# JohannesErnst/WeaSAL

Hardware: AMD Instinct MI355X
Metric: points/sec fwd+bwd KPFCNN on DALES spheres; achieved HBM GB/s on KPConv gather (higher is better)
Workload: dtype f32; 1 GPU; DALES_PseudoLabel KP-FCNN, in_radius=10m, 50k pts/sphere, batch=8, fp32, step = GPU pyramid + fwd + loss + bwd + SGD; contrast_loss term included (trainer_PseudoLabel.py:204-208); pyramid of the next batch overlapped on a second stream; parallelism=dp1, dist_world_size=1, allreduce_bytes=0

## Files before the change

### weasal_amd/csrc/pools.hip

```cpp
#include "ws_common.h"
#include <algorithm>
#include "ws_dispatch.h"

namespace {

__device__ __forceinline__ int64_t ws_ceil_div_dev(int64_t a, int64_t b) { return (a + b - 1) / b; }
bool al16p(const void* p) { return (reinterpret_cast<uintptr_t>(p) & 15u) == 0; }
__device__ __forceinline__ int4 load_arg4(const int32_t* p) { return *reinterpret_cast<const int4*>(p); }
__device__ __forceinline__ int4 load_arg4(const uint8_t* p)
{
    const unsigned w = *reinterpret_cast<const unsigned*>(p);
    return make_int4((int)(w & 0xffu), (int)((w >> 8) & 0xffu), (int)((w >> 16) & 0xffu), (int)(w >> 24));
}

__device__ __forceinline__ void pool_groups(int64_t ngroups, int ilv, int wave, int64_t& g0, int64_t& gstep, int64_t& gend)
{
    if (ilv > 0 && (gridDim.x & 7) == 0) {
        const int x = blockIdx.x & 7, lb = blockIdx.x >> 3, nbx = gridDim.x >> 3;
        const int64_t per8 = (ngroups + 7) / 8;
        const int64_t b8 = (int64_t)x * per8;
        gend = b8 + per8 < ngroups ? b8 + per8 : ngroups;
        g0 = b8 + (int64_t)lb * 4 + wave;
        gstep = (int64_t)nbx * 4;
    } else {
        int64_t ibeg, iend;
        ws_block_range(ngroups, ibeg, iend);
        g0 = ibeg + wave; gstep = 4; gend = iend;
    }
}

template <int G, typename T, typename AT = int32_t, int U = 4>
__global__ __launch_bounds__(256) void max_pool_fwd_vec_kernel(const T* __restrict__ x, int64_t ns, int c,
                                                                const int64_t* __restrict__ inds, int64_t nq, int h,
                                                                T* __restrict__ out, AT* __restrict__ arg,
                                                                const int32_t* __restrict__ order = nullptr, int ilv = 0, int split = 1)
{
    constexpr int S = 64 / G;
    const int wave = __builtin_amdgcn_readfirstlane(threadIdx.x >> 6), lane = threadIdx.x & 63;
    const int j = lane % G, slot = lane / G;
    int64_t g0, gstep, gend;
    pool_groups(ws_ceil_div_dev(nq, S) * split, ilv, wave, g0, gstep, gend);
    for (int64_t grp = g0; grp < gend; grp += gstep) {
        const int64_t qi = (grp / split) * S + slot;
        const bool qok = qi < nq;
        const int64_t q = (qok && order) ? (int64_t)order[qi] : qi;
        const int cbeg = split > 1 ? (int)(grp % split) * (4 * G) : 0;
        const int cend = split > 1 ? min(cbeg + 4 * G, c) : c;
        for (int c0 = cbeg; c0 < cend; c0 += 4 * G) {
            const int ch = c0 + 4 * j;
            const bool ok = qok && ch < c;
            float4 best = make_float4(-3.4e38f, -3.4e38f, -3.4e38f, -3.4e38f);
            int bi[4] = {0, 0, 0, 0};
            for (int h0 = 0; h0 < h; h0 += U) {
                float4 v[U];
#pragma unroll
                for (int u = 0; u < U; ++u) {
                    v[u] = make_float4(0.f, 0.f, 0.f, 0.f);
                    const int col = h0 + u;
                    int64_t s = (ok && col < h) ? inds[q * h + col] : -1;
                    if (s >= 0 && s < ns) v[u] = ld4(x + s * c + ch);
                    else if (col >= h) v[u] = make_float4(-3.4e38f, -3.4e38f, -3.4e38f, -3.4e38f);
                }
#pragma unroll
                for (int u = 0; u < U; ++u) {
                    if (v[u].x > best.x) { best.x = v[u].x; bi[0] = h0 + u; }
                    if (v[u].y > best.y) { best.y = v[u].y; bi[1] = h0 + u; }
                    if (v[u].z > best.z) { best.z = v[u].z; bi[2] = h0 + u; }
                    if (v[u].w > best.w) { best.w = v[u].w; bi[3] = h0 + u; }
                }
            }
            if (ok) {
                st4(out + q * c + ch, best);
                if (arg) {
                    if constexpr (sizeof(AT) == 4)
                        *reinterpret_cast<int4*>(arg + q * c + ch) = make_int4(bi[0], bi[1], bi[2], bi[3]);
                    else
                        *reinterpret_cast<unsigned*>(arg + q * c + ch) =
                            (unsigned)bi[0] | ((unsigned)bi[1] << 8) | ((unsigned)bi[2] << 16) | ((unsigned)bi[3] << 24);
                }
            }
        }
    }
}

template <typename T>
__global__ __launch_bounds__(256) void max_pool_fwd_kernel(const T* __restrict__ x, int64_t ns, int c,
                                                            const int64_t* __restrict__ inds, int64_t nq, int h,
                                                            T* __restrict__ out, int32_t* __restrict__ arg)
{
    const int wave = __builtin_amdgcn_readfirstlane(threadIdx.x >> 6), lane = threadIdx.x & 63;
    for (int64_t q = (int64_t)blockIdx.x * 4 + wave; q < nq; q += (int64_t)gridDim.x * 4) {
        for (int c0 = 0; c0 < c; c0 += 64) {
            const int ch = c0 + lane;
            float best = -3.4e38f;
            int bi = 0;
            for (int j = 0; j < h; ++j) {
                const int64_t s = inds[q * h + j];
                float v = 0.0f;
                if (s >= 0 && s < ns && ch < c) v = ld1(x + s * c + ch);
                if (v > best) { best = v; bi = j; }
            }
            if (ch < c) {
                st1(out + q * c + ch, best);
                if (arg) arg[q * c + ch] = bi;
            }
        }
    }
}

template <int G, typename T, typename AT = int32_t>
__global__ __launch_bounds__(256) void max_pool_bwd_vec_kernel(const T* __restrict__ dy, const AT* __restrict__ arg,
                                                                int h, int c, const int32_t* __restrict__ t_offsets,
                                                                const int32_t* __restrict__ t_pairs, int64_t ns,
                                                                T* __restrict__ dx, const int32_t* __restrict__ order = nullptr,
                                                                int ilv = 0, const T* __restrict__ add = nullptr, int split = 1)
{
    constexpr int S = 64 / G;
    const int wave = __builtin_amdgcn_readfirstlane(threadIdx.x >> 6), lane = threadIdx.x & 63;
    const int j = lane % G, slot = lane / G;
    int64_t g0, gstep, gend;
    pool_groups(ws_ceil_div_dev(ns, S) * split, ilv, wave, g0, gstep, gend);
    for (int64_t grp = g0; grp < gend; grp += gstep) {
        const int64_t si = (grp / split) * S + slot;
        const bool sok = si < ns;
        const int64_t s = (sok && order) ? (int64_t)order[si] : si;
        const int beg = sok ? t_offsets[s] : 0, end = sok ? t_offsets[s + 1] : 0;
        const int cbeg = split > 1 ? (int)(grp % split) * (4 * G) : 0;
        const int cend = split > 1 ? min(cbeg + 4 * G, c) : c;
        for (int c0 = cbeg; c0 < cend; c0 += 4 * G) {
            const int ch = c0 + 4 * j;
            if (!(sok && ch < c)) continue;
            float4 acc = make_float4(0.f, 0.f, 0.f, 0.f);
            int p = beg;
            for (; p + 3 < end; p += 4) {
                int q4[4], col4[4];
                int4 a4[4];
#pragma unroll
                for (int u = 0; u < 4; ++u) {
                    const int pair = t_pairs[p + u];
                    q4[u] = pair / h;
                    col4[u] = pair - q4[u] * h;
                }
#pragma unroll
                for (int u = 0; u < 4; ++u) a4[u] = load_arg4(arg + (int64_t)q4[u] * c + ch);
#pragma unroll
                for (int u = 0; u < 4; ++u) {
                    const int4 a = a4[u];
                    const int col = col4[u];
                    if (a.x == col || a.y == col || a.z == col || a.w == col) {
                        const float4 g = ld4(dy + (int64_t)q4[u] * c + ch);
                        if (a.x == col) acc.x += g.x;
                        if (a.y == col) acc.y += g.y;
                        if (a.z == col) acc.z += g.z;
                        if (a.w == col) acc.w += g.w;
                    }
                }
            }
            for (; p < end; ++p) {
                const int pair = t_pairs[p];
                const int q = pair / h, col = pair - q * h;
                const int4 a = load_arg4(arg + (int64_t)q * c + ch);
                if (a.x == col || a.y == col || a.z == col || a.w == col) {
                    const float4 g = ld4(dy + (int64_t)q * c + ch);
                    if (a.x == col) acc.x += g.x;
                    if (a.y == col) acc.y += g.y;
                    if (a.z == col) acc.z += g.z;
                    if (a.w == col) acc.w += g.w;
                }
            }
            if (add) { const float4 o = ld4(add + s * c + ch); acc.x += o.x; acc.y += o.y; acc.z += o.z; acc.w += o.w; }
            st4(dx + s * c + ch, acc);
        }
    }
}

template <typename T>
__global__ __launch_bounds__(256) void max_pool_bwd_kernel(const T* __restrict__ dy, const int32_t* __restrict__ arg,
                                                            int h, int c, const int32_t* __restrict__ t_offsets,
                                                            const int32_t* __restrict__ t_pairs, int64_t ns,
                                                            T* __restrict__ dx)
{
    const int wave = __builtin_amdgcn_readfirstlane(threadIdx.x >> 6), lane = threadIdx.x & 63;
    for (int64_t s = (int64_t)blockIdx.x * 4 + wave; s < ns; s += (int64_t)gridDim.x * 4) {
        const int beg = t_offsets[s], end = t_offsets[s + 1];
        for (int c0 = 0; c0 < c; c0 += 64) {
            const int ch = c0 + lane;
            float acc = 0.0f;
            if (ch < c) {
                for (int p = beg; p < end; ++p) {
                    const int pair = t_pairs[p];
                    const int q = pair / h, col = pair - q * h;
                    if (arg[(int64_t)q * c + ch] == col) acc += ld1(dy + (int64_t)q * c + ch);
                }
                st1(dx + s * c + ch, acc);
            }
        }
    }
}

template <typename T>
__global__ __launch_bounds__(256) void closest_pool_fwd_kernel(const T* __restrict__ x, int64_t ns, int c,
                                                                const int64_t* __restrict__ inds, int64_t nq, int h,
                                                                T* __restrict__ out)
{
    const int wave = __builtin_amdgcn_readfirstlane(threadIdx.x >> 6), lane = threadIdx.x & 63;
    for (int64_t q = (int64_t)blockIdx.x * 4 + wave; q < nq; q += (int64_t)gridDim.x * 4) {
        const int64_t s = inds[q * h];
        const bool real = s >= 0 && s < ns;
        for (int ch = lane; ch < c; ch += 64) st1(out + q * c + ch, real ? ld1(x + s * c + ch) : 0.0f);
    }
}

template <typename T>
__global__ __launch_bounds__(256) void closest_pool_bwd_kernel(const T* __restrict__ dy, int h, int c,
                                                                const int32_t* __restrict__ t_offsets,
                                                                const int32_t* __restrict__ t_pairs, int64_t ns,
                                                                T* __restrict__ dx)
{
    const int wave = __builtin_amdgcn_readfirstlane(threadIdx.x >> 6), lane = threadIdx.x & 63;
    for (int64_t s = (int64_t)blockIdx.x * 4 + wave; s < ns; s += (int64_t)gridDim.x * 4) {
        const int beg = t_offsets[s], end = t_offsets[s + 1];
        for (int c0 = 0; c0 < c; c0 += 64) {
            const int ch = c0 + lane;
            float acc = 0.0f;
            if (ch < c) {
                for (int p = beg; p < end; ++p) {
                    const int pair = t_pairs[p];
                    const int q = pair / h;
                    if (pair - q * h == 0) acc += ld1(dy + (int64_t)q * c + ch);
                }
                st1(dx + s * c + ch, acc);
            }
        }
    }
}


template <int G>
__global__ __launch_bounds__(256) void closest_pool_bwd_vec_kernel(const float* __restrict__ dy, int h, int c,
                                                                    const int32_t* __restrict__ t_offsets,
                                                                    const int32_t* __restrict__ t_pairs, int64_t ns,
                                                                    float* __restrict__ dx)
{
    constexpr int S = 64 / G;
    const int wave = __builtin_amdgcn_readfirstlane(threadIdx.x >> 6), lane = threadIdx.x & 63;
    const int j = lane % G, slot = lane / G;
    for (int64_t s = (int64_t)blockIdx.x * 4 + wave; s < ns; s += (int64_t)gridDim.x * 4) {
        const int beg = t_offsets[s], end = t_offsets[s + 1];
        for (int c0 = 0; c0 < c; c0 += 4 * G) {
            const int ch = c0 + 4 * j;
            float4 acc = make_float4(0.f, 0.f, 0.f, 0.f);
            int p = beg + slot;
            for (; p + S < end; p += 2 * S) {
                const int pa = t_pairs[p], pb = t_pairs[p + S];
                const int qa = pa / h, qb = pb / h;
                float4 a = make_float4(0.f, 0.f, 0.f, 0.f), b4 = a;
                if (pa - qa * h == 0) a = *reinterpret_cast<const float4*>(dy + (int64_t)qa * c + ch);
                if (pb - qb * h == 0) b4 = *reinterpret_cast<const float4*>(dy + (int64_t)qb * c + ch);
                acc.x += a.x; acc.y += a.y; acc.z += a.z; acc.w += a.w;
                acc.x += b4.x; acc.y += b4.y; acc.z += b4.z; acc.w += b4.w;
            }
            if (p < end) {
                const int pa = t_pairs[p];
                const int qa = pa / h;
                if (pa - qa * h == 0) {
                    const float4 a = *reinterpret_cast<const float4*>(dy + (int64_t)qa * c + ch);
                    acc.x += a.x; acc.y += a.y; acc.z += a.z; acc.w += a.w;
                }
            }
#pragma unroll
            for (int o = G; o < 64; o <<= 1) {
                acc.x += __shfl_xor(acc.x, o, 64); acc.y += __shfl_xor(acc.y, o, 64);
                acc.z += __shfl_xor(acc.z, o, 64); acc.w += __shfl_xor(acc.w, o, 64);
            }
            if (slot == 0) *reinterpret_cast<float4*>(dx + s * c + ch) = acc;
        }
    }
}

constexpr int POOL_INTERLEAVE = 256;
constexpr int POOL_SPLIT_ROWS = 8192;
extern "C" int ws_closest_bwd_vec = 1;

enum { PK_MAX_FWD_VEC, PK_MAX_FWD, PK_MAX_BWD_VEC, PK_MAX_BWD, PK_CLOSEST_FWD, PK_CLOSEST_BWD, PK_CLOSEST_BWD_VEC };
struct PoolPlan {
    int kernel;
    bool bf16;
    int g;
    int u;
    int arg_bytes;
    int split;
    int ilv;
    int grid;
};
const char* row_name(const PoolPlan& p) { return p.bf16 ? "bf16" : "f32"; }

int pool_grid(int64_t groups, int ilv)
{
    if (ilv <= 0) return ws_grid(groups, 4);
    const int64_t need = (groups + 31) / 32;
    return 8 * (int)std::max<int64_t>(1, std::min<int64_t>(ilv, need));
}

PoolPlan max_pool_plan(bool fwd, bool bf16, int64_t rows, int c, const void* a, const void* b, const void* arg, int arg_bytes, bool ordered)
{
    PoolPlan p{fwd ? PK_MAX_FWD : PK_MAX_BWD, bf16, 0, 0, arg_bytes, 1, 0, ws_grid(rows, 4)};
    const bool rows_al = bf16 ? ws_row_aligned<bf16_t>(a) && ws_row_aligned<bf16_t>(b) : ws_row_aligned<float>(a) && ws_row_aligned<float>(b);
    if (arg_bytes != 1 && !(c % 4 == 0 && rows_al && al16p(arg))) return p;
    p.kernel = fwd ? PK_MAX_FWD_VEC : PK_MAX_BWD_VEC;
    p.g = (fwd && c <= 16) ? 4 : (c <= 32 ? 8 : (c <= 64 ? 16 : (c <= 128 ? 32 : 64)));
    p.u = (fwd && arg_bytes == 1 && p.g == 32) ? 8 : 4;
    p.split = (rows < POOL_SPLIT_ROWS && c > 256) ? (int)ws_ceil_div(c, 256) : 1;
    p.ilv = ordered ? POOL_INTERLEAVE : 0;
    p.grid = pool_grid(ws_ceil_div(rows, 64 / p.g) * p.split, p.ilv);
    return p;
}

PoolPlan closest_fwd_plan(bool bf16, int64_t nq) { return PoolPlan{PK_CLOSEST_FWD, bf16, 0, 0, 0, 1, 0, ws_grid(nq, 4)}; }

PoolPlan closest_bwd_plan(bool bf16, int64_t ns, int c, const void* dy, const void* dx)
{
    PoolPlan p{PK_CLOSEST_BWD, bf16, 0, 0, 0, 1, 0, ws_grid(ns, 4)};
    if (!bf16 && ws_closest_bwd_vec && al16p(dy) && al16p(dx) && (c == 32 || c == 64 || c == 128 || c % 256 == 0)) {
        p.kernel = PK_CLOSEST_BWD_VEC;
        p.g = c % 256 == 0 ? 64 : c / 4;
    }
    return p;
}

void plan_text(const PoolPlan& p, char* out, size_t n)
{
    const char* op = (p.kernel == PK_MAX_FWD_VEC || p.kernel == PK_MAX_FWD) ? "max_fwd" : "max_bwd";
    switch (p.kernel) {
    case PK_MAX_FWD_VEC: case PK_MAX_BWD_VEC:
        snprintf(out, n, "%s vec G=%d U=%d AT=%s %s split=%d %s", op, p.g, p.u, p.arg_bytes == 1 ? "u8" : "i32", row_name(p), p.split,
                 p.ilv ? "interleaved" : "contiguous");
        break;
    case PK_MAX_FWD: case PK_MAX_BWD: snprintf(out, n, "%s generic %s", op, row_name(p)); break;
    case PK_CLOSEST_FWD: snprintf(out, n, "closest_fwd scalar %s", row_name(p)); break;
    case PK_CLOSEST_BWD: snprintf(out, n, "closest_bwd scalar %s", row_name(p)); break;
    default: snprintf(out, n, "closest_bwd vec G=%d", p.g);
    }
}

int launched(bool hit, const PoolPlan& p)
{
    if (!hit) return ws_no_instantiation("pool kernel family %d <G=%d, U=%d> bf16=%d arg_bytes=%d", p.kernel, p.g, p.u, p.bf16, p.arg_bytes);
    WS_LAUNCH_CHECK();
    return WS_OK;
}

int launch_fwd(const PoolPlan& p, void* stream, const void* x, int64_t ns, int32_t c, const int64_t* inds, int64_t nq, int32_t h, void* out,
               void* arg, const int32_t* order)
{
    hipStream_t st = (hipStream_t)stream;
    bool hit = false;
    if (p.kernel == PK_MAX_FWD_VEC)
        dispatch([&](auto bf, auto g, auto u, auto u8) {
            using T = Row<bf.value>;
            using AT = std::conditional_t<u8.value != 0, uint8_t, int32_t>;
            if constexpr (!(bf.value && u8.value) && (u.value == 8) == (u8.value && g.value == 32)) {
                max_pool_fwd_vec_kernel<g.value, T, AT, u.value><<<p.grid, 256, 0, st>>>((const T*)x, ns, c, inds, nq, h, (T*)out, (AT*)arg, order,
                                                                                         p.ilv, p.split);
                hit = true;
            }
        }, Flag{p.bf16}, Pick<4, 8, 16, 32, 64>{p.g}, Pick<4, 8>{p.u}, Flag{p.arg_bytes == 1});
    else
        hit = dispatch([&](auto bf) {
            using T = Row<bf.value>;
            if (p.kernel == PK_MAX_FWD) max_pool_fwd_kernel<T><<<p.grid, 256, 0, st>>>((const T*)x, ns, c, inds, nq, h, (T*)out, (int32_t*)arg);
            else closest_pool_fwd_kernel<T><<<p.grid, 256, 0, st>>>((const T*)x, ns, c, inds, nq, h, (T*)out);
        }, Flag{p.bf16});
    return launched(hit, p);
}

int launch_bwd(const PoolPlan& p, void* stream, const void* dy, const void* arg, int32_t h, int32_t c, const int32_t* t_offsets,
               const int32_t* t_pairs, int64_t ns, void* dx, const int32_t* order, const float* add = nullptr)
{
    hipStream_t st = (hipStream_t)stream;
    bool hit = false;
    if (p.kernel == PK_MAX_BWD_VEC)
        dispatch([&](auto bf, auto g, auto u8) {
            using T = Row<bf.value>;
            using AT = std::conditional_t<u8.value != 0, uint8_t, int32_t>;
            if constexpr (!(bf.value && u8.value)) {
                max_pool_bwd_vec_kernel<g.value, T, AT><<<p.grid, 256, 0, st>>>((const T*)dy, (const AT*)arg, h, c, t_offsets, t_pairs, ns, (T*)dx,
                                                                                order, p.ilv, (const T*)add, p.split);
                hit = true;
            }
        }, Flag{p.bf16}, Pick<8, 16, 32, 64>{p.g}, Flag{p.arg_bytes == 1});
    else if (p.kernel == PK_CLOSEST_BWD_VEC)
        hit = dispatch([&](auto g) {
            closest_pool_bwd_vec_kernel<g.value><<<p.grid, 256, 0, st>>>((const float*)dy, h, c, t_offsets, t_pairs, ns, (float*)dx);
        }, Pick<8, 16, 32, 64>{p.g});
    else
        hit = dispatch([&](auto bf) {
            using T = Row<bf.value>;
            if (p.kernel == PK_MAX_BWD) max_pool_bwd_kernel<T><<<p.grid, 256, 0, st>>>((const T*)dy, (const int32_t*)arg, h, c, t_offsets, t_pairs, ns, (T*)dx);
            else closest_pool_bwd_kernel<T><<<p.grid, 256, 0, st>>>((const T*)dy, h, c, t_offsets, t_pairs, ns, (T*)dx);
        }, Flag{p.bf16});
    return launched(hit, p);
}

int pool_fwd_impl(bool closest, bool bf16, const void* x, int64_t ns, int32_t c, const int64_t* inds, int64_t nq, int32_t h, void* out,
                  int32_t* arg, const int32_t* order, void* stream)
{
    WS_REQUIRE(ns >= 0 && nq >= 0 && c >= 1 && h >= 1, "bad sizes");
    if (nq == 0) return WS_OK;
    WS_REQUIRE(inds && out && (ns == 0 || x), "NULL argument");
    const PoolPlan p = closest ? closest_fwd_plan(bf16, nq) : max_pool_plan(true, bf16, nq, c, x, out, arg, 4, order != nullptr);
    return launch_fwd(p, stream, x, ns, c, inds, nq, h, out, arg, order);
}

int pool_bwd_impl(bool closest, bool bf16, const void* dy, const int32_t* arg, int64_t nq, int32_t h, int32_t c, const int32_t* t_offsets,
                  const int32_t* t_pairs, int64_t ns, void* dx, const int32_t* order, void* stream)
{
    WS_REQUIRE(ns >= 0 && nq >= 0 && c >= 1 && h >= 1, "bad sizes");
    if (ns == 0) return WS_OK;
    WS_REQUIRE(t_offsets && dx && (nq == 0 || (dy && (closest || arg) && t_pairs)), "NULL argument");
    const PoolPlan p = closest ? closest_bwd_plan(bf16, ns, c, dy, dx) : max_pool_plan(false, bf16, ns, c, dy, dx, arg, 4, order != nullptr);
    return launch_bwd(p, stream, dy, arg, h, c, t_offsets, t_pairs, ns, dx, order);
}

}

extern "C" {

int ws_max_pool_fwd(const float* x, int64_t ns, int32_t c, const int64_t* inds, int64_t nq, int32_t h,
                    float* out, int32_t* arg, void* stream)
{
    return pool_fwd_impl(false, false, x, ns, c, inds, nq, h, out, arg, nullptr, stream);
}

int ws_max_pool_bwd(const float* dy, const int32_t* arg, int64_t nq, int32_t h, int32_t c,
                    const int32_t* t_offsets, const int32_t* t_pairs, int64_t ns, float* dx, void* stream)
{
    return pool_bwd_impl(false, false, dy, arg, nq, h, c, t_offsets, t_pairs, ns, dx, nullptr, stream);
}

int ws_max_pool_fwd_ordered(const float* x, int64_t ns, int32_t c, const int64_t* inds, int64_t nq, int32_t h, float* out, int32_t* arg,
                            const int32_t* order_q, void* stream)
{
    return pool_fwd_impl(false, false, x, ns, c, inds, nq, h, out, arg, order_q, stream);
}

int ws_max_pool_bwd_ordered(const float* dy, const int32_t* arg, int64_t nq, int32_t h, int32_t c, const int32_t* t_offsets,
                            const int32_t* t_pairs, int64_t ns, float* dx, const int32_t* order_s, void* stream)
{
    return pool_bwd_impl(false, false, dy, arg, nq, h, c, t_offsets, t_pairs, ns, dx, order_s, stream);
}

int ws_max_pool_fwd_ordered_bf16(const uint16_t* x, int64_t ns, int32_t c, const int64_t* inds, int64_t nq, int32_t h, uint16_t* out,
                                 int32_t* arg, const int32_t* order_q, void* stream)
{
    return pool_fwd_impl(false, true, x, ns, c, inds, nq, h, out, arg, order_q, stream);
}

int ws_max_pool_bwd_ordered_bf16(const uint16_t* dy, const int32_t* arg, int64_t nq, int32_t h, int32_t c, const int32_t* t_offsets,
                                 const int32_t* t_pairs, int64_t ns, uint16_t* dx, const int32_t* order_s, void* stream)
{
    return pool_bwd_impl(false, true, dy, arg, nq, h, c, t_offsets, t_pairs, ns, dx, order_s, stream);
}

int ws_closest_pool_fwd(const float* x, int64_t ns, int32_t c, const int64_t* inds, int64_t nq, int32_t h,
                        float* out, void* stream)
{
    return pool_fwd_impl(true, false, x, ns, c, inds, nq, h, out, nullptr, nullptr, stream);
}

int ws_closest_pool_bwd(const float* dy, int64_t nq, int32_t h, int32_t c, const int32_t* t_offsets,
                        const int32_t* t_pairs, int64_t ns, float* dx, void* stream)
{
    return pool_bwd_impl(true, false, dy, nullptr, nq, h, c, t_offsets, t_pairs, ns, dx, nullptr, stream);
}

int ws_max_pool_fwd_bf16(const uint16_t* x, int64_t ns, int32_t c, const int64_t* inds, int64_t nq, int32_t h,
                         uint16_t* out, int32_t* arg, void* stream)
{
    return pool_fwd_impl(false, true, x, ns, c, inds, nq, h, out, arg, nullptr, stream);
}

int ws_max_pool_bwd_bf16(const uint16_t* dy, const int32_t* arg, int64_t nq, int32_t h, int32_t c,
                         const int32_t* t_offsets, const int32_t* t_pairs, int64_t ns, uint16_t* dx, void* stream)
{
    return pool_bwd_impl(false, true, dy, arg, nq, h, c, t_offsets, t_pairs, ns, dx, nullptr, stream);
}

int ws_closest_pool_fwd_bf16(const uint16_t* x, int64_t ns, int32_t c, const int64_t* inds, int64_t nq, int32_t h,
                             uint16_t* out, void* stream)
{
    return pool_fwd_impl(true, true, x, ns, c, inds, nq, h, out, nullptr, nullptr, stream);
}

int ws_closest_pool_bwd_bf16(const uint16_t* dy, int64_t nq, int32_t h, int32_t c, const int32_t* t_offsets,
                             const int32_t* t_pairs, int64_t ns, uint16_t* dx, void* stream)
{
    return pool_bwd_impl(true, true, dy, nullptr, nq, h, c, t_offsets, t_pairs, ns, dx, nullptr, stream);
}

int ws_priv_max_pool_fwd_u8(const float* x, int64_t ns, int32_t c, const int64_t* inds, int64_t nq, int32_t h, float* out,
                            uint8_t* arg, const int32_t* order_q, void* stream)
{
    if (nq == 0) return WS_OK;
    return launch_fwd(max_pool_plan(true, false, nq, c, x, out, arg, 1, order_q != nullptr), stream, x, ns, c, inds, nq, h, out, arg, order_q);
}

int ws_priv_max_pool_bwd_u8(const float* dy, const uint8_t* arg, int64_t nq, int32_t h, int32_t c, const int32_t* t_offsets,
                            const int32_t* t_pairs, int64_t ns, float* dx, const int32_t* order_s, const float* add, void* stream)
{
    (void)nq;
    if (ns == 0) return WS_OK;
    return launch_bwd(max_pool_plan(false, false, ns, c, dy, dx, arg, 1, order_s != nullptr), stream, dy, arg, h, c, t_offsets, t_pairs, ns,
                          dx, order_s, add);
}

int ws_pool_variant(int32_t op, int64_t rows, int32_t c, const void* rows_a, const void* rows_b, const void* arg, int32_t rows_bf16,
                    int32_t arg_bytes, int32_t ordered, char* out, int32_t cap, int32_t* grid)
{
    WS_REQUIRE(out && cap > 0 && rows >= 0 && c >= 1 && (arg_bytes == 4 || arg_bytes == 1), "bad argument");
    const bool bf = rows_bf16 != 0, max_op = op == WS_POOL_MAX_FWD || op == WS_POOL_MAX_BWD;
    WS_REQUIRE(arg_bytes == 4 || (max_op && !bf && c % 4 == 0 && al16p(rows_a) && al16p(rows_b) && (reinterpret_cast<uintptr_t>(arg) & 3u) == 0),
               "the byte arg-max record: max-pools of f32 rows, c %% 4 == 0, 16-byte aligned rows, 4-byte aligned arg");
    PoolPlan p;
    switch (op) {
    case WS_POOL_MAX_FWD: case WS_POOL_MAX_BWD: p = max_pool_plan(op == WS_POOL_MAX_FWD, bf, rows, c, rows_a, rows_b, arg, arg_bytes, ordered != 0); break;
    case WS_POOL_CLOSEST_FWD: p = closest_fwd_plan(bf, rows); break;
    case WS_POOL_CLOSEST_BWD: p = closest_bwd_plan(bf, rows, c, rows_a, rows_b); break;
    default: return ws_fail(WS_ERR_INVALID, "unknown pool operation %d", op);
    }
    plan_text(p, out, (size_t)cap);
    if (grid) *grid = p.grid;
    return WS_OK;
}

}
```

Before: 32.61 million points/s.

## Software-pipeline pair/offset loads and shuffle-broadcast pairs in pool backward kernels

Result: no change. 32.88 million points/s (median of 3 runs) (+0.8%).

```diff
diff --git a/weasal_amd/csrc/pools.hip b/weasal_amd/csrc/pools.hip
--- a/weasal_amd/csrc/pools.hip
+++ b/weasal_amd/csrc/pools.hip
@@ -6,12 +6,6 @@
 
 __device__ __forceinline__ int64_t ws_ceil_div_dev(int64_t a, int64_t b) { return (a + b - 1) / b; }
 bool al16p(const void* p) { return (reinterpret_cast<uintptr_t>(p) & 15u) == 0; }
-__device__ __forceinline__ int4 load_arg4(const int32_t* p) { return *reinterpret_cast<const int4*>(p); }
-__device__ __forceinline__ int4 load_arg4(const uint8_t* p)
-{
-    const unsigned w = *reinterpret_cast<const unsigned*>(p);
-    return make_int4((int)(w & 0xffu), (int)((w >> 8) & 0xffu), (int)((w >> 16) & 0xffu), (int)(w >> 24));
-}
 
 __device__ __forceinline__ void pool_groups(int64_t ngroups, int ilv, int wave, int64_t& g0, int64_t& gstep, int64_t& gend)
 {
@@ -108,69 +102,112 @@
     }
 }
 
-template <int G, typename T, typename AT = int32_t>
+__device__ __forceinline__ int4 load_argp(const int32_t* p) { return *reinterpret_cast<const int4*>(p); }
+__device__ __forceinline__ unsigned load_argp(const uint8_t* p) { return *reinterpret_cast<const unsigned*>(p); }
+__device__ __forceinline__ int argp_ch(const int4& a, int i) { return i == 0 ? a.x : (i == 1 ? a.y : (i == 2 ? a.z : a.w)); }
+__device__ __forceinline__ int argp_ch(unsigned w, int i) { return (int)((w >> (8 * i)) & 0xffu); }
+template <typename P>
+__device__ __forceinline__ bool argp_any(const P& a, int col)
+{
+    return argp_ch(a, 0) == col || argp_ch(a, 1) == col || argp_ch(a, 2) == col || argp_ch(a, 3) == col;
+}
+__device__ __forceinline__ void split_pair(int pair, int h, int& q, int& col)
+{
+    q = 0; col = -1;
+    if (pair >= 0) { q = pair / h; col = pair - q * h; }
+}
+
+constexpr int POOL_BWD_BATCH = 4;
+
+template <int G, typename T, typename AT = int32_t, int B = (sizeof(AT) == 1 ? POOL_BWD_BATCH : POOL_BWD_BATCH / 2)>
 __global__ __launch_bounds__(256) void max_pool_bwd_vec_kernel(const T* __restrict__ dy, const AT* __restrict__ arg,
                                                                 int h, int c, const int32_t* __restrict__ t_offsets,
                                                                 const int32_t* __restrict__ t_pairs, int64_t ns,
                                                                 T* __restrict__ dx, const int32_t* __restrict__ order = nullptr,
                                                                 int ilv = 0, const T* __restrict__ add = nullptr, int split = 1)
 {
+    static_assert(G % B == 0, "a batch never straddles a pair chunk");
     constexpr int S = 64 / G;
     const int wave = __builtin_amdgcn_readfirstlane(threadIdx.x >> 6), lane = threadIdx.x & 63;
     const int j = lane % G, slot = lane / G;
     int64_t g0, gstep, gend;
     pool_groups(ws_ceil_div_dev(ns, S) * split, ilv, wave, g0, gstep, gend);
+
+    auto slot_si = [&](int64_t g) -> int64_t {
+        const int64_t si = (split > 1 ? g / split : g) * S + slot;
+        return (g < gend && si < ns) ? si : -1;
+    };
+    auto ld_order = [&](int64_t g) -> int { const int64_t si = slot_si(g); return (order && si >= 0) ? order[si] : 0; };
+    auto row_of = [&](int64_t g, int ov) -> int64_t { const int64_t si = slot_si(g); return (order && si >= 0) ? (int64_t)ov : si; };
+    auto ld_offsets = [&](int64_t s, int& b, int& e) { b = e = 0; if (s >= 0) { b = t_offsets[s]; e = t_offsets[s + 1]; } };
+    auto ld_chunk = [&](int b, int e, int k0) -> int { return k0 + j < e - b ? t_pairs[b + k0 + j] : -1; };
+
+    int o0 = ld_order(g0), o1 = ld_order(g0 + gstep), o2 = ld_order(g0 + 2 * gstep);
+    int b0, e0, b1, e1;
+    ld_offsets(row_of(g0, o0), b0, e0);
+    ld_offsets(row_of(g0 + gstep, o1), b1, e1);
+    int pw0 = ld_chunk(b0, e0, 0);
     for (int64_t grp = g0; grp < gend; grp += gstep) {
-        const int64_t si = (grp / split) * S + slot;
-        const bool sok = si < ns;
-        const int64_t s = (sok && order) ? (int64_t)order[si] : si;
-        const int beg = sok ? t_offsets[s] : 0, end = sok ? t_offsets[s + 1] : 0;
+        const int o3 = ld_order(grp + 3 * gstep);
+        int b2, e2;
+        ld_offsets(row_of(grp + 2 * gstep, o2), b2, e2);
+        const int pw1 = ld_chunk(b1, e1, 0);
+
+        const int64_t s = row_of(grp, o0);
+        const int deg = e0 - b0;
+        int pq0, pc0;
+        split_pair(pw0, h, pq0, pc0);
         const int cbeg = split > 1 ? (int)(grp % split) * (4 * G) : 0;
         const int cend = split > 1 ? min(cbeg + 4 * G, c) : c;
         for (int c0 = cbeg; c0 < cend; c0 += 4 * G) {
             const int ch = c0 + 4 * j;
-            if (!(sok && ch < c)) continue;
+            const bool act = s >= 0 && ch < c;
             float4 acc = make_float4(0.f, 0.f, 0.f, 0.f);
-            int p = beg;
-            for (; p + 3 < end; p += 4) {
-                int q4[4], col4[4];
-                int4 a4[4];
-#pragma unroll
-                for (int u = 0; u < 4; ++u) {
-                    const int pair = t_pairs[p + u];
-                    q4[u] = pair / h;
-                    col4[u] = pair - q4[u] * h;
-                }
-#pragma unroll
-                for (int u = 0; u < 4; ++u) a4[u] = load_arg4(arg + (int64_t)q4[u] * c + ch);
-#pragma unroll
-                for (int u = 0; u < 4; ++u) {
-                    const int4 a = a4[u];
-                    const int col = col4[u];
-                    if (a.x == col || a.y == col || a.z == col || a.w == col) {
-                        const float4 g = ld4(dy + (int64_t)q4[u] * c + ch);
-                        if (a.x == col) acc.x += g.x;
-                        if (a.y == col) acc.y += g.y;
-                        if (a.z == col) acc.z += g.z;
-                        if (a.w == col) acc.w += g.w;
+            for (int k0 = 0; k0 < deg; k0 += G) {
+                int pq = pq0, pc = pc0;
+                if (k0 > 0) split_pair(ld_chunk(b0, e0, k0), h, pq, pc);
+                const int n = min(deg - k0, G);
+                for (int k = 0; k < n; k += B) {
+                    int q[B], col[B];
+                    decltype(load_argp(arg)) a[B];
+                    float4 g[B];
+                    bool m[B];
+#pragma unroll
+                    for (int u = 0; u < B; ++u) {
+                        q[u] = __shfl(pq, k + u, G);
+                        const int cu = __shfl(pc, k + u, G);
+                        col[u] = act ? cu : -1;
                     }
-                }
-            }
-            for (; p < end; ++p) {
-                const int pair = t_pairs[p];
-                const int q = pair / h, col = pair - q * h;
-                const int4 a = load_arg4(arg + (int64_t)q * c + ch);
-                if (a.x == col || a.y == col || a.z == col || a.w == col) {
-                    const float4 g = ld4(dy + (int64_t)q * c + ch);
-                    if (a.x == col) acc.x += g.x;
-                    if (a.y == col) acc.y += g.y;
-                    if (a.z == col) acc.z += g.z;
-                    if (a.w == col) acc.w += g.w;
-                }
-            }
-            if (add) { const float4 o = ld4(add + s * c + ch); acc.x += o.x; acc.y += o.y; acc.z += o.z; acc.w += o.w; }
-            st4(dx + s * c + ch, acc);
+#pragma unroll
+                    for (int u = 0; u < B; ++u) {
+                        a[u] = decltype(load_argp(arg)){};
+                        if (col[u] >= 0) a[u] = load_argp(arg + (int64_t)q[u] * c + ch);
+                    }
+#pragma unroll
+                    for (int u = 0; u < B; ++u) {
+                        m[u] = col[u] >= 0 && argp_any(a[u], col[u]);
+                        g[u] = make_float4(0.f, 0.f, 0.f, 0.f);
+                        if (m[u]) g[u] = ld4(dy + (int64_t)q[u] * c + ch);
+                    }
+#pragma unroll
+                    for (int u = 0; u < B; ++u) {
+                        if (m[u]) {
+                            if (argp_ch(a[u], 0) == col[u]) acc.x += g[u].x;
+                            if (argp_ch(a[u], 1) == col[u]) acc.y += g[u].y;
+                            if (argp_ch(a[u], 2) == col[u]) acc.z += g[u].z;
+                            if (argp_ch(a[u], 3) == col[u]) acc.w += g[u].w;
+                        }
+                    }
+                }
+            }
+            if (act) {
+                if (add) { const float4 o = ld4(add + s * c + ch); acc.x += o.x; acc.y += o.y; acc.z += o.z; acc.w += o.w; }
+                st4(dx + s * c + ch, acc);
+            }
         }
+        o0 = o1; o1 = o2; o2 = o3;
+        b0 = b1; e0 = e1; b1 = b2; e1 = e2;
+        pw0 = pw1;
     }
 }
 
@@ -245,27 +282,40 @@
     constexpr int S = 64 / G;
     const int wave = __builtin_amdgcn_readfirstlane(threadIdx.x >> 6), lane = threadIdx.x & 63;
     const int j = lane % G, slot = lane / G;
-    for (int64_t s = (int64_t)blockIdx.x * 4 + wave; s < ns; s += (int64_t)gridDim.x * 4) {
-        const int beg = t_offsets[s], end = t_offsets[s + 1];
+    const int64_t s0 = (int64_t)blockIdx.x * 4 + wave, sstep = (int64_t)gridDim.x * 4;
+    auto ld_offsets = [&](int64_t s, int& b, int& e) { b = e = 0; if (s < ns) { b = t_offsets[s]; e = t_offsets[s + 1]; } };
+    auto ld_chunk = [&](int b, int e, int k0) -> int { return k0 + lane < e - b ? t_pairs[b + k0 + lane] : -1; };
+    auto dy_row = [&](int pair) -> int {
+        if (pair < 0) return -1;
+        const int q = pair / h;
+        return pair - q * h == 0 ? q : -1;
+    };
+    int b0, e0, b1, e1;
+    ld_offsets(s0, b0, e0);
+    ld_offsets(s0 + sstep, b1, e1);
+    int pw0 = ld_chunk(b0, e0, 0);
+    for (int64_t s = s0; s < ns; s += sstep) {
+        int b2, e2;
+        ld_offsets(s + 2 * sstep, b2, e2);
+        const int pw1 = ld_chunk(b1, e1, 0);
+        const int deg = e0 - b0;
+        const int r0 = dy_row(pw0);
         for (int c0 = 0; c0 < c; c0 += 4 * G) {
             const int ch = c0 + 4 * j;
             float4 acc = make_float4(0.f, 0.f, 0.f, 0.f);
-            int p = beg + slot;
-            for (; p + S < end; p += 2 * S) {
-                const int pa = t_pairs[p], pb = t_pairs[p + S];
-                const int qa = pa / h, qb = pb / h;
-                float4 a = make_float4(0.f, 0.f, 0.f, 0.f), b4 = a;
-                if (pa - qa * h == 0) a = *reinterpret_cast<const float4*>(dy + (int64_t)qa * c + ch);
-                if (pb - qb * h == 0) b4 = *reinterpret_cast<const float4*>(dy + (int64_t)qb * c + ch);
-                acc.x += a.x; acc.y += a.y; acc.z += a.z; acc.w += a.w;
-                acc.x += b4.x; acc.y += b4.y; acc.z += b4.z; acc.w += b4.w;
-            }
-            if (p < end) {
-                const int pa = t_pairs[p];
-                const int qa = pa / h;
-                if (pa - qa * h == 0) {
-                    const float4 a = *reinterpret_cast<const float4*>(dy + (int64_t)qa * c + ch);
-                    acc.x += a.x; acc.y += a.y; acc.z += a.z; acc.w += a.w;
+            for (int k0 = 0; k0 < deg; k0 += 64) {
+                const int r = k0 == 0 ? r0 : dy_row(ld_chunk(b0, e0, k0));
+                const int n = min(deg - k0, 64);
+                for (int i = 0; i * S < n; i += 4) {
+                    float4 v[4];
+#pragma unroll
+                    for (int u = 0; u < 4; ++u) {
+                        const int ru = __shfl(r, slot + (i + u) * S, 64);
+                        v[u] = make_float4(0.f, 0.f, 0.f, 0.f);
+                        if (ru >= 0) v[u] = *reinterpret_cast<const float4*>(dy + (int64_t)ru * c + ch);
+                    }
+#pragma unroll
+                    for (int u = 0; u < 4; ++u) { acc.x += v[u].x; acc.y += v[u].y; acc.z += v[u].z; acc.w += v[u].w; }
                 }
             }
 #pragma unroll
@@ -275,6 +325,8 @@
             }
             if (slot == 0) *reinterpret_cast<float4*>(dx + s * c + ch) = acc;
         }
+        b0 = b1; e0 = e1; b1 = b2; e1 = e2;
+        pw0 = pw1;
     }
 }
 
```
